# dell-research-harvard/effocr

Hardware: AMD Instinct MI355X
Metric: glyph-crops/sec end-to-end (encode+kNN), 224x224 bs=1024 (higher is better)
Workload: dtype bf16; 1 GPU; BASELINE configs[1]: vit_small_patch16_224 encoder (bf16 MFMA operands, fp32 accumulate/residual/LN/softmax), 1024x3x224x224 fp32 crops per GPU resident in HBM, 10000-row fp32 IndexFlatIP, k=10; seeded random-init weights; crops_per_gpu=1024, global_batch=1024, index_rows=10000, k=10, parallelism=1024 crops per GPU, weights+index replicated

## Files before the change

### effocr_amd/csrc/api.hip

```cpp
#include "../../include/effocr_hip.h"
#include "enc_core.hpp"


#include <math.h>
#include <algorithm>
#include <string.h>
#include <map>
#include <memory>
#include <string>
#include <vector>

namespace effocr {

namespace {

struct Param { std::string name; std::vector<int64_t> shape; int64_t numel; std::vector<float> data; bool set; };

struct VitCfg { int D, depth, heads, mlp; };
struct VitLayerOff { size_t ln1w, ln1b, qkvb, projb, ln2w, ln2b, fc1b, fc2b, qkvw, projw, fc1w, fc2w;
                     size_t qkvw_b, projw_b, fc1w_b, fc2w_b, projw_pp, fc2w_pp, projb_p, fc2b_p, qkvw_bv, qkvb_v;
                     size_t qkvw_bf, qkv_s, qkv_c, fc1w_bf, fc1_s, fc1_c; };
struct ConvSpec { std::string w, bn; int cin, cout, k, stride, pad; size_t w_off, b_off; };
struct CnxBlockOff { size_t dww, dwb, lnw, lnb, w1, b1, w2, b2, gamma; };
struct CnxStageOff { int C, Cp, depth; size_t dslnw, dslnb, dsw, dsb; std::vector<CnxBlockOff> blocks; };

}
}

using namespace effocr;

struct effocr_encoder {
  std::string arch;
  bool is_vit = false;
  int img = 224, prec = PREC_BF16, D = 0;
  std::vector<Param> params;
  std::map<std::string, int> index;
  VitCfg vit{};
  int T = 0, P = 0;
  size_t off_clspos0 = 0, off_pos = 0, off_patchb = 0, off_normw = 0, off_normb = 0, off_patchw = 0, off_patchw_b = 0;
  std::vector<VitLayerOff> layers;
  std::vector<ConvSpec> convs;
  bool is_cnx = false;
  std::vector<CnxStageOff> cnx;
  size_t cnx_stemw = 0, cnx_stemb = 0, cnx_stemlnw = 0, cnx_stemlnb = 0, cnx_headw = 0, cnx_headb = 0;
  bool is_mnv = false;
  MnvNet mnv{};
  size_t wbytes = 0;
  const char* wdev = nullptr;
  int debug = 0;
  int cls_only_last = 1;
  int mlp_stagger_min_rounds = 2;
  int mlp_tail_first = 96;
  int mlp_stagger = 2500;
  int use_projf = 1;
  int use_qkvattn = 1;
  int qa_min_batch = 1;
  int qa_hsplit = 0;
  int use_patchf = 1;
  int use_mlp = 1;
  int use_gemm3 = 1;
  int use_lnfold = 1;
  int tail_split = 1;
  int split6 = 1;
  int pair_parts = 1;
  int mlp_pair = 0;
  int use_blocked = 1;
  int use_gemm2 = 1;
  int panel_rows = 128;
  int use_panel = 1;
  int chunk = 0;
  int call_size_invariant = 0;
  int prof_mode = 0;
  std::string prof_only;
  std::vector<std::pair<hipEvent_t, hipEvent_t>> prof_pool;
  std::vector<std::pair<int, int>> prof_rec;
  std::vector<std::string> prof_names;
  size_t prof_used = 0;
  std::vector<float> prof_ms;
  std::vector<int> prof_cnt;
  std::vector<double> prof_work;
  unsigned long long* prof_clk = nullptr;
  std::vector<double> prof_ghz;
  static constexpr size_t PROF_CLK_SLOTS = 256;
};

namespace effocr {
namespace {

int64_t prod(const std::vector<int64_t>& s) { int64_t p = 1; for (auto v : s) p *= v; return p; }

void add_param(effocr_encoder* e, const std::string& name, std::vector<int64_t> shape) {
  Param p; p.name = name; p.shape = shape; p.numel = prod(shape); p.set = false;
  e->index[name] = (int)e->params.size();
  e->params.push_back(std::move(p));
}

void build_vit(effocr_encoder* e) {
  const int D = e->vit.D, depth = e->vit.depth, mlp = e->vit.mlp;
  e->P = (e->img / 16) * (e->img / 16);
  e->T = e->P + 1;
  add_param(e, "cls_token", {1, 1, D});
  add_param(e, "pos_embed", {1, e->T, D});
  add_param(e, "patch_embed.proj.weight", {D, 3, 16, 16});
  add_param(e, "patch_embed.proj.bias", {D});
  for (int i = 0; i < depth; ++i) {
    const std::string p = "blocks." + std::to_string(i) + ".";
    add_param(e, p + "norm1.weight", {D});
    add_param(e, p + "norm1.bias", {D});
    add_param(e, p + "attn.qkv.weight", {3 * D, D});
    add_param(e, p + "attn.qkv.bias", {3 * D});
    add_param(e, p + "attn.proj.weight", {D, D});
// ... 455 lines not shown
}

struct VitWs { size_t status, x, xn, qkv, att, h, stats, total, rows, hbytes; };
VitWs vit_ws(const effocr_encoder* e, int B) {
  const size_t M = align_up((size_t)B * e->T, 128), D = e->vit.D, es = prec_esize(e->prec);
  Alloc a; VitWs w;
  w.rows = M;
  w.status = a.take(256);
  w.x = a.take(M * D * 4);
  w.xn = a.take(M * D * es);
  w.qkv = a.take(M * 3 * D * es);
  w.att = a.take(M * D * es);
  size_t hb = M * e->vit.mlp * es, pb = (size_t)B * e->P * 768 * es;
  w.hbytes = hb > pb ? hb : pb;
  {
    const size_t cus = (size_t)device_cus(), np = M / 128, tail = np % cus;
    const size_t split = (tail && tail * 6 <= cus) ? 6 : (tail && tail * 4 <= cus) ? 4 : (tail && tail * 2 <= cus) ? 2 : 0;
    const size_t need = split * tail * 128 * D * 4;
    if (need > w.hbytes) w.hbytes = need;
  }
  w.h = a.take(w.hbytes);
  w.stats = a.take(M * 64);
  w.total = a.off;
  return w;
}

int vit_forward(effocr_encoder* e, const void* x, int x16, int B, float* emb, int l2, char* ws, hipStream_t s) {
  const VitWs w = vit_ws(e, B);
  const int D = e->vit.D, T = e->T, Pn = e->P, M = B * T, prec = e->prec;
  const char* wb = e->wdev;
  float* xs = reinterpret_cast<float*>(ws + w.x);
  void* xn = ws + w.xn; void* qkv = ws + w.qkv; void* att = ws + w.att; void* hb = ws + w.h;
  auto F = [&](size_t off) { return reinterpret_cast<const float*>(wb + off); };
  int rc;
  const double Md = (double)M, Dd = (double)D, Hd = (double)e->vit.mlp;
  const bool panel = e->use_panel && panel_gemm_supported(prec, 3 * D, D) && panel_gemm_supported(prec, e->vit.mlp, D);
  const bool g2 = e->use_gemm2 && gemm2_supported(prec, D, e->vit.mlp);
  const bool g2p = e->use_gemm2 && gemm2_supported(prec, D, 768);
  const bool g3all = !panel && e->use_gemm3 && gemm3_supported(prec, 3 * D, D) && gemm3_supported(prec, D, D) &&
                     gemm3_supported(prec, e->vit.mlp, D) && gemm3_supported(prec, D, e->vit.mlp);
  const int blk = (e->use_blocked && g2p && ((panel && g2) || g3all)) ? 1 : 0;
  const bool mlpf = blk && panel && e->use_mlp && mlp_fused_supported(prec, D, e->vit.mlp);
  const bool projf = mlpf && e->use_projf;
  const bool qaf = blk && panel && mlpf && qkv_attn_supported(prec, D, T) && (e->use_qkvattn == 2 || (e->use_qkvattn == 1 && (e->call_size_invariant || B >= e->qa_min_batch)));
  const bool g3 = blk && e->use_gemm3 && gemm3_supported(prec, D, e->vit.mlp);
  const bool patchf = blk && e->use_patchf && patch_embed_fused_supported(prec, D);
  if (!patchf && (rc = timed(e, "im2col_patch16", 0.0, s, [&] { return im2col_patch16(prec, x, x16, B, e->img, e->img, hb, s); }))) return rc;
  int* status = reinterpret_cast<int*>(ws + w.status);
  if (!patchf && (rc = set_cls_rows(F(e->off_clspos0), xs, B, T, D, blk, nullptr, s))) return rc;
  GemmArgs g{};
  if (patchf) {
    PatchArgs pa{};
    pa.x = x; pa.x16 = x16; pa.B = B; pa.H = e->img; pa.W = e->img; pa.Wb = wb + e->off_patchw_b; pa.bias = F(e->off_patchb); pa.pos = F(e->off_pos);
    pa.out = xs; pa.D = D; pa.P = Pn; pa.cls = F(e->off_clspos0);
    if ((rc = timed(e, "patch_embed_fused", 2.0 * B * Pn * Dd * 768.0, s, [&] { return patch_embed_fused(prec, pa, s); }))) return rc;
  } else {
  g.X = hb; g.ldx = 768; g.W = wb + e->off_patchw; g.ldw = 768; g.bias = F(e->off_patchb);
  g.out = xs; g.ldo = D; g.pos = F(e->off_pos); g.M = B * Pn; g.N = D; g.K = 768; g.P = Pn; g.blk_out = blk;
  if ((rc = timed(e, "gemm_patch_embed", 2.0 * B * Pn * Dd * 768.0, s, [&] { return g2p ? gemm2_nt(prec, EPI_PATCH, g, s) : gemm_nt(prec, EPI_PATCH, g, s); }))) return rc;
  }
  const float* cls_x = nullptr;
  bool xn_ready = false;
  for (int i = 0; i < e->vit.depth; ++i) {
    const VitLayerOff& L = e->layers[i];
    if (panel) {
      {
      PanelArgs p{};
      if (qaf) {
        if (!xn_ready && (rc = timed(e, "layernorm", 0.0, s, [&] { return layernorm_rows_blocked(prec, xs, M, D, F(L.ln1w), F(L.ln1b), 1e-6f, xn, s); }))) return rc;
        xn_ready = false;
        QkvAttnArgs q{};
        q.xn = xn; q.Wb = wb + L.qkvw_bv; q.bias = F(L.qkvb_v); q.out = att;
        q.B = B; q.T = T; q.D = D; q.rows_alloc = (int64_t)w.rows; q.hsplit = e->qa_hsplit;
        q.cls_only = (i + 1 == e->vit.depth && e->cls_only_last && projf) ? 1 : 0;
        const bool cls_k = q.cls_only && D == 384 && T > 192;
        const double qa_work = cls_k ? 2.0 * Md * 2.0 * Dd * Dd + 2.0 * (32.0 * B) * Dd * Dd + 4.0 * B * e->vit.heads * 32.0 * T * 64.0
                                     : 2.0 * Md * 3.0 * Dd * Dd + 4.0 * B * e->vit.heads * (double)T * T * 64.0;
        if ((rc = timed(e, "qkv_attn_fused", qa_work, s, [&] { return qkv_attn_fused(prec, q, s); }))) return rc;
      } else {
      p.A = xs; p.lda = D; p.gamma = F(L.ln1w); p.beta = F(L.ln1b); p.eps = 1e-6f; p.W = wb + L.qkvw; p.bias = F(L.qkvb);
      p.out = qkv; p.ldo = 3 * D; p.M = M; p.N = 3 * D; p.K = D; p.rows_padded = 1; p.debug = e->debug; p.panel_rows = e->panel_rows; p.no_tail_split = !e->tail_split;
      p.blk_a = blk; p.blk_out = blk;
      if ((rc = timed(e, "panel_ln_qkv", 2.0 * Md * 3.0 * Dd * Dd, s, [&] { return panel_gemm(prec, PRO_LN, EPI_BIAS, p, s); }))) return rc;
      if ((rc = timed(e, "attention", 4.0 * B * e->vit.heads * (double)T * T * 64.0, s, [&] { return attention(prec, qkv, att, B, T, e->vit.heads, blk, s); }))) return rc;
      }
      if (!projf) {
      p = PanelArgs{};
      p.A = att; p.lda = D; p.W = wb + L.projw; p.bias = F(L.projb); p.out = xs; p.ldo = D; p.resid = xs; p.ldr = D;
      p.M = M; p.N = D; p.K = D; p.rows_padded = 1; p.debug = e->debug; p.panel_rows = e->panel_rows; p.no_tail_split = !e->tail_split; p.blk_a = blk; p.blk_out = blk;
      if ((rc = timed(e, "panel_proj_resid", 2.0 * Md * Dd * Dd, s, [&] { return panel_gemm(prec, PRO_COPY, EPI_BIAS_RESID, p, s); }))) return rc;
      }
      }
      if (mlpf) {
        MlpArgs m{};
        m.x = xs; m.gamma = F(L.ln2w); m.beta = F(L.ln2b); m.eps = 1e-6f; m.W1b = wb + L.fc1w_b; m.b1 = F(L.fc1b);
        m.W2p = wb + L.fc2w_pp; m.b2 = F(L.fc2b_p); m.b2_logical = F(L.fc2b); m.M = M; m.D = D; m.H = e->vit.mlp; m.rows_alloc = (int)w.rows;
        m.partial = reinterpret_cast<float*>(hb); m.partial_bytes = w.hbytes; m.no_tail_split = !e->tail_split; m.no_split6 = !e->split6; m.pair = e->mlp_pair; m.no_pair_parts = !e->pair_parts; m.stagger = e->mlp_stagger; m.stagger_min_rounds = e->mlp_stagger_min_rounds; m.tail_first = e->mlp_tail_first;
        if (e->call_size_invariant) { m.no_tail_split = 1; m.pair = -1; }
        if (projf) {
          m.A = att; m.Wpp = wb + L.projw_pp; m.bp = F(L.projb_p);
          if (i + 1 == e->vit.depth && e->cls_only_last) {
            const size_t Bp = align_up((size_t)B, 128);
            float* xc = reinterpret_cast<float*>(qkv);
            void* ac = static_cast<char*>(qkv) + Bp * D * 4;
            if ((rc = timed(e, "gather_cls", 0.0, s, [&] { return gather_cls_rows_blocked(xs, att, B, T, D, xc, ac, s); }))) return rc;
            m.x = xc; m.A = ac; m.M = B; m.rows_alloc = (int)Bp;
            const double Bd = B;
// ... 363 lines not shown
  auto it = enc->index.find(name);
  if (it == enc->index.end()) return fail(EFFOCR_EINVAL, std::string("set_param: unknown parameter '") + name + "'");
  Param& p = enc->params[it->second];
  if (p.numel != numel)
    return fail(EFFOCR_EINVAL, std::string("set_param: '") + name + "' expects " + std::to_string(p.numel) +
                                   " elements, got " + std::to_string(numel));
  p.data.assign(host, host + numel);
  p.set = true;
  return EFFOCR_OK;
}

size_t effocr_encoder_weights_bytes(const effocr_encoder_t* enc) { return enc ? enc->wbytes : 0; }

int effocr_encoder_upload(effocr_encoder_t* enc, void* weights_dev, size_t bytes) {
  if (!enc || !weights_dev) return fail(EFFOCR_EINVAL, "upload: NULL argument");
  if (bytes < enc->wbytes) return fail(EFFOCR_EWORKSPACE, "upload: weight buffer too small");
  for (const Param& p : enc->params)
    if (!p.set) return fail(EFFOCR_ESTATE, "upload: parameter '" + p.name + "' was never set");
  std::vector<char> blob(enc->wbytes, 0);
  if (enc->is_vit) pack_vit(enc, blob); else if (enc->is_cnx) pack_convnext(enc, blob); else if (enc->is_mnv) pack_mobilenetv3(enc, blob);
  else pack_resnet(enc, blob);
  const hipError_t er = hipMemcpy(weights_dev, blob.data(), enc->wbytes, hipMemcpyHostToDevice);
  if (er != hipSuccess) return fail(EFFOCR_EHIP, std::string("upload: hipMemcpy: ") + hipGetErrorString(er));
  enc->wdev = static_cast<const char*>(weights_dev);
  return EFFOCR_OK;
}

size_t effocr_encoder_workspace_bytes(const effocr_encoder_t* enc, int batch) {
  if (!enc || batch <= 0) return 0;
  if (enc->is_cnx) return convnext_ws(enc, cnx_chunk(enc, batch)).total;
  if (enc->is_mnv) return mnv3_ws(enc, mnv3_chunk(enc, batch)).total;
  if (!enc->is_vit) return resnet_ws(enc, batch).total;
  return vit_ws(enc, (enc->chunk > 0 && enc->chunk < batch) ? enc->chunk : batch).total;
}

int effocr_encoder_set_option(effocr_encoder_t* enc, const char* name, int value) {
  if (!enc || !name) return fail(EFFOCR_EINVAL, "set_option: NULL argument");
  const std::string n = name;
  if (n == "use_panel") { enc->use_panel = value; return EFFOCR_OK; }
  if (n == "debug") { enc->debug = value; return EFFOCR_OK; }
  if (n == "use_gemm2") { enc->use_gemm2 = value; return EFFOCR_OK; }
  if (n == "use_blocked") { enc->use_blocked = value; return EFFOCR_OK; }
  if (n == "tail_split") { enc->tail_split = value; return EFFOCR_OK; }
  if (n == "split6") { enc->split6 = value; return EFFOCR_OK; }
  if (n == "mlp_pair") { enc->mlp_pair = value; return EFFOCR_OK; }
  if (n == "pair_parts") { enc->pair_parts = value; return EFFOCR_OK; }
  if (n == "use_gemm3") { enc->use_gemm3 = value; return EFFOCR_OK; }
  if (n == "use_lnfold") { enc->use_lnfold = value; return EFFOCR_OK; }
  if (n == "use_mlp") { enc->use_mlp = value; return EFFOCR_OK; }
  if (n == "use_qkvattn") { enc->use_qkvattn = value; return EFFOCR_OK; }
  if (n == "qa_min_batch") { enc->qa_min_batch = value; return EFFOCR_OK; }
  if (n == "qa_hsplit") { enc->qa_hsplit = value; return EFFOCR_OK; }
  if (n == "use_patchf") { enc->use_patchf = value; return EFFOCR_OK; }
  if (n == "use_projf") { enc->use_projf = value; return EFFOCR_OK; }
  if (n == "cls_only_last") { enc->cls_only_last = value; return EFFOCR_OK; }
  if (n == "mlp_stagger_min_rounds") { enc->mlp_stagger_min_rounds = value < 1 ? 1 : value; return EFFOCR_OK; }
  if (n == "mlp_tail_first") { enc->mlp_tail_first = value < 0 ? 0 : value & ~7; return EFFOCR_OK; }
  if (n == "mlp_stagger") { enc->mlp_stagger = value < 0 ? 0 : value; return EFFOCR_OK; }
  if (n == "panel_rows") { if (value != 64 && value != 128) return fail(EFFOCR_EINVAL, "set_option: panel_rows must be 64 or 128"); enc->panel_rows = value; return EFFOCR_OK; }
  if (n == "call_size_invariant") {
    if (value != 0 && value != 1) return fail(EFFOCR_EINVAL, "set_option: call_size_invariant must be 0 or 1");
    enc->call_size_invariant = value; return EFFOCR_OK;
  }
  if (n == "chunk") { if (value < 0) return fail(EFFOCR_EINVAL, "set_option: chunk < 0"); enc->chunk = value; return EFFOCR_OK; }
  return fail(EFFOCR_EINVAL, "set_option: unknown option '" + n + "'");
}

int effocr_encoder_set_chunk(effocr_encoder_t* enc, int crops_per_chunk) {
  if (!enc || crops_per_chunk < 0) return fail(EFFOCR_EINVAL, "set_chunk: bad argument");
  enc->chunk = crops_per_chunk;
  return EFFOCR_OK;
}

int effocr_encoder_forward(effocr_encoder_t* enc, const float* x_dev, int batch, float* emb_dev, int l2_normalize,
                           void* workspace_dev, size_t workspace_bytes, void* stream) {
  return effocr_encoder_forward_ex(enc, x_dev, EFFOCR_PREC_FP32, batch, emb_dev, l2_normalize, workspace_dev, workspace_bytes, stream);
}

int effocr_encoder_forward_ex(effocr_encoder_t* enc, const void* x_dev, int x_dtype, int batch, float* emb_dev, int l2_normalize,
                              void* workspace_dev, size_t workspace_bytes, void* stream) {
  if (!enc) return fail(EFFOCR_EINVAL, "forward: NULL encoder");
  if (x_dtype != PREC_FP32 && !(enc->is_vit && enc->prec != PREC_FP32 && x_dtype == enc->prec))
    return fail(x_dtype < 0 || x_dtype > 2 ? EFFOCR_EINVAL : EFFOCR_EUNSUPPORTED,
                "forward: crops must be fp32, or (ViT, 16-bit precision modes) already in the encoder's own operand type");
  const int x16 = x_dtype != PREC_FP32;
  if (batch < 0) return fail(EFFOCR_EINVAL, "forward: negative batch");
  if (batch == 0) return EFFOCR_OK;
  if (!x_dev || !emb_dev || !workspace_dev) return fail(EFFOCR_EINVAL, "forward: NULL device pointer");
  if (!enc->wdev) return fail(EFFOCR_ESTATE, "forward: weights were not uploaded");
  if (workspace_bytes < effocr_encoder_workspace_bytes(enc, batch)) return fail(EFFOCR_EWORKSPACE, "forward: workspace too small");
  if ((int64_t)batch * (enc->is_vit ? enc->T : enc->img * enc->img) >= (int64_t)1 << 30)
    return fail(EFFOCR_EUNSUPPORTED, "forward: batch too large for 32-bit row indices");
  char* ws = static_cast<char*>(workspace_dev);
  if (enc->is_cnx) {
    const int chunk = cnx_chunk(enc, batch);
    const int64_t so = enc->img / 4;
    if ((int64_t)chunk * so * so * 4 * enc->cnx[0].C >= (int64_t)1 << 31)
      return fail(EFFOCR_EUNSUPPORTED, "forward: chunk too large for 32-bit GEMM row indices (effocr_encoder_set_chunk)");
    const size_t img_bytes = (size_t)3 * enc->img * enc->img * 4;
    for (int b0 = 0; b0 < batch; b0 += chunk) {
      const int cb = (batch - b0 < chunk) ? batch - b0 : chunk;
      const int rc = convnext_forward(enc, reinterpret_cast<const float*>(static_cast<const char*>(x_dev) + (size_t)b0 * img_bytes), cb,
                                      emb_dev + (size_t)b0 * enc->D, l2_normalize, ws, S(stream));
      if (rc) return rc;
    }
    return EFFOCR_OK;
// ... 319 lines not shown
```

### effocr_amd/csrc/kernels.hpp

```cpp
#pragma once
#include "common.hpp"

namespace effocr {

enum { PREC_BF16 = 0, PREC_FP16 = 1, PREC_FP32 = 2 };
enum { EPI_BIAS = 0, EPI_BIAS_GELU = 1, EPI_BIAS_RESID = 2, EPI_PATCH = 3,
       EPI_BIAS_SCALE_RESID = 4,
       EPI_BIAS_F32 = 5 };

static inline int prec_esize(int prec) { return prec == PREC_FP32 ? 4 : 2; }

struct GemmArgs {
  const void* X; int64_t ldx;
  const void* W; int64_t ldw;
  const float* bias;
  void* out; int64_t ldo;
  const float* resid; int64_t ldr;
  const float* pos;
  int M, N, K;
  int P;
  int blk_x;
  int blk_out;
  const void* Wblk;
  int rows_alloc;
// ... 5 lines not shown

int gemm_nt(int prec, int epi, const GemmArgs& g, hipStream_t s);

bool gemm2_supported(int prec, int N, int K);
int gemm2_nt(int prec, int epi, const GemmArgs& g, hipStream_t s);

bool gemm3_supported(int prec, int N, int K);
bool gemm3_lnfold_supported(int D);
int gemm3_nt(int prec, int epi, const GemmArgs& g, hipStream_t s);

struct MlpArgs {
  float* x;
  const float* gamma; const float* beta; float eps;
  const void* W1b; const float* b1;
  const void* W2p; const float* b2;
  int M, D, H;
  int rows_alloc;
  float* partial; size_t partial_bytes;
  int no_tail_split;
  int no_split6;
  int no_pair_parts;
  int pair;
  int panel0, tail_rb, stagger_wgs, main_wgs;
  int stagger;
  int stagger_min_rounds;
  int tail_first;
  const void* A; const void* Wpp; const float* bp; const float* b2_logical;
  void* xn_out; const float* gamma_n; const float* beta_n;
};
bool mlp_fused_supported(int prec, int D, int H);
int mlp_fused(int prec, const MlpArgs& a, hipStream_t s);

struct QkvAttnArgs {
  const void* xn;
  const void* Wb; const float* bias;
  void* out;
  int B, T, D;
  int64_t rows_alloc;
  int cls_only;
  int img0;
  int hsplit;
};
bool qkv_attn_supported(int prec, int D, int T);
int qkv_attn_fused(int prec, const QkvAttnArgs& a, hipStream_t s);

struct PatchArgs {
  const void* x; int B, H, W;
  int x16;
  const void* Wb;
  const float* bias; const float* pos;
  const float* cls;
  float* out;
  int D, P;
};
bool patch_embed_fused_supported(int prec, int D);
int patch_embed_fused(int prec, const PatchArgs& a, hipStream_t s);

enum { PRO_COPY = 0, PRO_LN = 1 };
struct PanelArgs {
  const void* A; int64_t lda;
  const float* gamma; const float* beta; float eps;
  const void* W;
  const float* bias;
  void* out; int64_t ldo;
  const float* resid; int64_t ldr;
  int M, N, K;
  unsigned long long* dbg;
  int debug;
  int blk_a;
  int blk_out;
  int panel_rows;
  int rows_padded;
  int no_tail_split;
  int tail_first, tail_split;
};
bool panel_gemm_supported(int prec, int N, int K);
int panel_gemm(int prec, int pro, int epi, const PanelArgs& a, hipStream_t s);

int reduce_layernorm_rows_blocked(int prec_out, float* x, int64_t rows, int D, const float* partial, const float* b2, int nparts, int tail_rb,
                                  int add_x, const float* gamma, const float* beta, float eps, void* out, hipStream_t s);
int layernorm_rows_blocked(int prec_out, const float* x, int64_t rows, int D, const float* gamma, const float* beta,
                           float eps, void* out, hipStream_t s);
int layernorm_rows(int prec_out, const float* x, int64_t rows, int D, const float* gamma, const float* beta,
                   float eps, void* out, hipStream_t s);
int im2col_patch16(int prec_out, const void* x, int x16, int B, int H, int W, void* out, hipStream_t s);
int clock_sample(unsigned long long* out, hipStream_t s);
int set_cls_rows(const float* cls_pos0, float* x, int B, int T, int D, int blocked, int* status_zero, hipStream_t s);
int gather_cls_rows_blocked(const float* x, const void* att, int B, int T, int D, float* xc, void* ac, hipStream_t s);
int attention(int prec, const void* qkv, void* out, int B, int T, int heads, int blocked, hipStream_t s);
int final_cls_norm(const float* x, int B, int T, int D, const float* gamma, const float* beta, float eps,
                   int l2norm, int blocked, float* emb, int* status, hipStream_t s);

size_t knn_workspace_bytes(int64_t B, int64_t N, int D, int k);
int knn_ip_topk(const float* q, int64_t B, const float* xb, int64_t N, int D, int k, float* dist, int64_t* idx,
                void* ws, size_t ws_bytes, hipStream_t s);
size_t knn_screen_workspace_bytes(int64_t B, int64_t N, int D, int k);
void knn_set_wg_target(int n);
void knn_q16_tile(int on);
void knn_two_pass_screen(int on);
void knn_force_tile_kernel(int on);
size_t knn_screen_flag_offset(int64_t B, int64_t N, int D, int k);
int knn_ip_topk_screened(const float* q, int64_t B, const float* xb, const void* xb16, const void* xblk, int64_t N, int D, int k, float xnorm_max,
                         float* dist, int64_t* idx, void* ws, size_t ws_bytes, hipStream_t s);
int convert_bf16_blocked(const float* src, int64_t N, int D, void* dst, hipStream_t s);
void knn_qs_option(int which, int value);
int convert_bf16(const float* src, int64_t n, void* dst, hipStream_t s);
// ... 68 lines not shown
```

### effocr_amd/csrc/patch.hip

```cpp
#include "common.hpp"
#include "kernels.hpp"
#include <type_traits>

constexpr int PE_SLABS = 2;
constexpr int PE_SLABS16 = 4;
#ifndef PATCH_NT
#define PATCH_NT 1
#endif
namespace effocr {
namespace {

template <int I, int N, typename F> __device__ __forceinline__ void pfor(F&& f) {
  if constexpr (I < N) {
    f(std::integral_constant<int, I>{});
    pfor<I + 1, N>(f);
  }
}

constexpr int PE_STAGE = 16384;
constexpr int PE_RING = 8;
constexpr int PE_K = 768;

template <typename E, typename X, int D>
__global__ __launch_bounds__(256, 1) void patch_embed_kernel(PatchArgs a) {
  typedef typename Op16<E>::V8 V8;
  constexpr bool X16 = sizeof(X) == 2;
  constexpr int NSL = X16 ? PE_SLABS16 : PE_SLABS;
  constexpr int KC = PE_K / 8;
  constexpr int OT = D / 32, OG = OT / 4;
  constexpr int KS = PE_K / 64;
  constexpr int NS = KS * OG;
  constexpr int R = PE_RING;
  static_assert(D % 128 == 0 && D <= 384, "patch_embed: a workgroup's output slice must be 128, 256 or 384 wide");
  static_assert(NS >= R - 1, "patch_embed: the panel's stream must be at least as long as the prefetch distance");
  __shared__ __attribute__((aligned(16))) char smem[R * PE_STAGE];
  const int tid = threadIdx.x, lane = tid & 63, r31 = lane & 31, half = lane >> 5;
  const int w = wave_id();
  const int64_t total = (int64_t)a.B * a.P;
  const int nsl = a.D / D;
  const int panel = (int)blockIdx.x / nsl, n0 = ((int)blockIdx.x - panel * nsl) * D;
  const int64_t m = (int64_t)panel * 128 + w * 32 + r31;
  const int64_t mc = m < total ? m : total - 1;
  const int img = (int)(mc / a.P), p = (int)(mc - (int64_t)img * a.P);
  const int PW = a.W / 16, ty = p / PW, tx = p - ty * PW;
  const X* xp = static_cast<const X*>(a.x) + ((int64_t)img * 3 * a.H + ty * 16) * a.W + tx * 16 + 8 * half;
  const int64_t plane = (int64_t)a.H * a.W;

  struct Slab { u32x4 v[X16 ? 4 : 8]; };
  auto load_slab = [&](Slab& sl, int ks) __attribute__((always_inline)) {
#pragma unroll
    for (int c4 = 0; c4 < 4; ++c4) {
      const int kk = ks * 4 + c4;
      const X* q = xp + (int64_t)(kk >> 4) * plane + (int64_t)(kk & 15) * a.W;
      if constexpr (X16) {
        sl.v[c4] = (PATCH_NT & 1) ? __builtin_nontemporal_load(reinterpret_cast<const u32x4*>(q)) : *reinterpret_cast<const u32x4*>(q);
      } else {
        sl.v[2 * c4] = (PATCH_NT & 1) ? __builtin_nontemporal_load(reinterpret_cast<const u32x4*>(q)) : *reinterpret_cast<const u32x4*>(q);
        sl.v[2 * c4 + 1] = (PATCH_NT & 1) ? __builtin_nontemporal_load(reinterpret_cast<const u32x4*>(q + 4)) : *reinterpret_cast<const u32x4*>(q + 4);
      }
    }
  };
  Slab sl[NSL];
#pragma unroll
  for (int i = 0; i < NSL; ++i) load_slab(sl[i], i);
  asm volatile("" ::: "memory");

  const char* Wb = static_cast<const char*>(a.Wb);
  const unsigned lane16 = (unsigned)lane * 16u;
  auto stage_src = [&](int s) __attribute__((always_inline)) -> const char* {
    const int ks = s / OG, g = s - ks * OG;
    return Wb + ((size_t)(4 * g + w + (n0 >> 5)) * KC + 8 * ks) * 512 + lane16;
  };
  const unsigned sW_lds = (unsigned)(size_t)(__attribute__((address_space(3))) char*)smem;
#pragma unroll
  for (int s0 = 0; s0 < R - 1; ++s0) {
    const __attribute__((address_space(1))) void* src = (const __attribute__((address_space(1))) void*)stage_src(s0);
    __attribute__((address_space(3))) void* dst = (__attribute__((address_space(3))) void*)(smem + s0 * PE_STAGE + w * 4096);
    __builtin_amdgcn_global_load_lds(src, dst, 16, 0, 0);
    __builtin_amdgcn_global_load_lds(src, dst, 16, 1024, 0);
    __builtin_amdgcn_global_load_lds(src, dst, 16, 2048, 0);
    __builtin_amdgcn_global_load_lds(src, dst, 16, 3072, 0);
  }
  auto issue_stage_asm = [&](int s) __attribute__((always_inline)) {
    const char* src = stage_src(s);
    const unsigned dst = (unsigned)__builtin_amdgcn_readfirstlane((int)(sW_lds + (unsigned)((s & (R - 1)) * PE_STAGE) + (unsigned)w * 4096u));
    unsigned keep;
    asm volatile("s_mov_b32 %0, m0\n\t"
                 "s_mov_b32 m0, %2\n\t"
                 "s_nop 0\n\t"
                 "global_load_lds_dwordx4 %1, off\n\t"
                 "global_load_lds_dwordx4 %1, off offset:1024\n\t"
                 "global_load_lds_dwordx4 %1, off offset:2048\n\t"
                 "global_load_lds_dwordx4 %1, off offset:3072\n\t"
                 "s_mov_b32 m0, %0"
                 : "=&s"(keep) : "v"(src), "s"(dst) : "memory");
  };

  auto to_frags = [&](const Slab& sl, V8 (&xf)[4]) __attribute__((always_inline)) {
#pragma unroll
    for (int c4 = 0; c4 < 4; ++c4) {
      if constexpr (X16) xf[c4] = __builtin_bit_cast(V8, sl.v[c4]);
      else {
        const f32x4 lo = __builtin_bit_cast(f32x4, sl.v[2 * c4]), hi = __builtin_bit_cast(f32x4, sl.v[2 * c4 + 1]);
        const u32x2 p0 = pack4<E>(lo[0], lo[1], lo[2], lo[3]);
        const u32x2 p1 = pack4<E>(hi[0], hi[1], hi[2], hi[3]);
        const u32x4 q = {p0[0], p0[1], p1[0], p1[1]};
        xf[c4] = __builtin_bit_cast(V8, q);
      }
    }
  };

  f32x16 acc[OT];
#pragma unroll
  for (int t = 0; t < OT; ++t)
#pragma unroll
    for (int r = 0; r < 16; ++r) acc[t][r] = 0.f;

  V8 xf[4];

  const int wo = half * 512 + r31 * 16;
  struct WF { V8 w[4]; };
  WF wf;
  asm volatile("s_waitcnt vmcnt(%0)" ::"n"((R - 2) * 4) : "memory");
  __builtin_amdgcn_s_barrier();
  asm volatile("" ::: "memory");
#pragma unroll
  for (int i = 0; i < 4; ++i) wf.w[i] = *reinterpret_cast<const V8*>(smem + wo + (i * 8) * 512);

  pfor<0, NS>([&](auto S_) {
    constexpr int S = decltype(S_)::value;
    constexpr int ks = S / OG, g = S % OG;
    constexpr bool more = S + R - 1 < NS, next = S + 1 < NS;
    const char* st = smem + (S & (R - 1)) * PE_STAGE;
    const char* stn = smem + ((S + 1) & (R - 1)) * PE_STAGE;
    if constexpr (g == 0) {
      to_frags(sl[ks % NSL], xf);
      if constexpr (ks + NSL < KS) load_slab(sl[ks % NSL], ks + NSL);
    }
    pfor<0, 4>([&](auto C4) {
      constexpr int c4 = decltype(C4)::value;
      if constexpr (c4 == 2) {
        if constexpr (S + R - 2 < NS) asm volatile("s_waitcnt vmcnt(%0)" ::"n"((R - 3) * 4) : "memory");
        else asm volatile("s_waitcnt vmcnt(0)" ::: "memory");
        __builtin_amdgcn_s_barrier();
        asm volatile("" ::: "memory");
      }
      pfor<0, 4>([&](auto I) {
        constexpr int i = decltype(I)::value;
        acc[4 * g + i] = Op16<E>::mfma(wf.w[i], xf[c4], acc[4 * g + i]);
        __builtin_amdgcn_sched_barrier(0);
        if constexpr (c4 < 3) wf.w[i] = *reinterpret_cast<const V8*>(st + wo + (i * 8 + 2 * (c4 + 1)) * 512);
        else if constexpr (next) wf.w[i] = *reinterpret_cast<const V8*>(stn + wo + (i * 8) * 512);
        if constexpr (more && c4 == 2 && i == 0) issue_stage_asm(S + R - 1);
      });
    });
  });

  if (m < total) {
    const int64_t orow = (int64_t)img * (a.P + 1) + 1 + p;
    const float* posr = a.pos + (int64_t)(1 + p) * a.D + n0;
    const float* biasr = a.bias + n0;
    char* ob = reinterpret_cast<char*>(a.out) + ((orow >> 5) * (a.D >> 2) + (n0 >> 2)) * 512 + (orow & 31) * 16;
    pfor<0, OT>([&](auto T_) {
      constexpr int t = decltype(T_)::value;
#pragma unroll
      for (int q = 0; q < 4; ++q) {
        const int f0 = 32 * t + 8 * q + 4 * half;
        const f32x4 bv = *reinterpret_cast<const f32x4*>(biasr + f0);
        const f32x4 pv = *reinterpret_cast<const f32x4*>(posr + f0);
        const f32x4 o = {acc[t][4 * q] + bv[0] + pv[0], acc[t][4 * q + 1] + bv[1] + pv[1], acc[t][4 * q + 2] + bv[2] + pv[2],
                         acc[t][4 * q + 3] + bv[3] + pv[3]};
        if (PATCH_NT & 2) __builtin_nontemporal_store(o, reinterpret_cast<f32x4*>(ob + (f0 >> 2) * 512)); else *reinterpret_cast<f32x4*>(ob + (f0 >> 2) * 512) = o;
      }
    });
    if (a.cls != nullptr && p == 0) {
      const int64_t crow = orow - 1;
      char* cb = reinterpret_cast<char*>(a.out) + ((crow >> 5) * (a.D >> 2) + (n0 >> 2)) * 512 + (crow & 31) * 16;
      for (int c = half; c < D / 4; c += 2)
        *reinterpret_cast<f32x4*>(cb + c * 512) = *reinterpret_cast<const f32x4*>(a.cls + n0 + 4 * c);
    }
  }
}

template <typename E, typename X>
int launch_patch(const PatchArgs& a, hipStream_t s) {
  const int64_t total = (int64_t)a.B * a.P;
  const int64_t panels = (total + 127) / 128;
  if (a.D == 384 && panels * 3 <= device_cus()) {
    hipLaunchKernelGGL((patch_embed_kernel<E, X, 128>), dim3((unsigned)(panels * 3)), dim3(256), 0, s, a);
    return check_launch("patch_embed_fused");
  }
  const int nsl = a.D > 384 ? a.D / 384 : 1;
  const dim3 grid((unsigned)(panels * nsl)), blk(256);
  switch (a.D) {
    case 128: hipLaunchKernelGGL((patch_embed_kernel<E, X, 128>), grid, blk, 0, s, a); break;
    case 256: hipLaunchKernelGGL((patch_embed_kernel<E, X, 256>), grid, blk, 0, s, a); break;
    case 384: case 768: hipLaunchKernelGGL((patch_embed_kernel<E, X, 384>), grid, blk, 0, s, a); break;
    default: return fail(EFFOCR_EUNSUPPORTED, "patch_embed_fused: embed dim must be 128, 256, 384 or 768");
  }
  return check_launch("patch_embed_fused");
}

}

bool patch_embed_fused_supported(int prec, int D) { return (prec == PREC_BF16 || prec == PREC_FP16) && (D == 128 || D == 256 || D == 384 || D == 768); }

int patch_embed_fused(int prec, const PatchArgs& a, hipStream_t s) {
  if (a.B <= 0) return EFFOCR_OK;
  if (!patch_embed_fused_supported(prec, a.D)) return fail(EFFOCR_EUNSUPPORTED, "patch_embed_fused: needs bf16/fp16 and an embed dim of 128, 256, 384 or 768");
  if (a.H % 16 || a.W % 16 || a.P != (a.H / 16) * (a.W / 16)) return fail(EFFOCR_EINVAL, "patch_embed_fused: image size must be a multiple of 16");
  if (a.x16) return prec == PREC_BF16 ? launch_patch<__bf16, __bf16>(a, s) : launch_patch<_Float16, _Float16>(a, s);
  return prec == PREC_BF16 ? launch_patch<__bf16, float>(a, s) : launch_patch<_Float16, float>(a, s);
}

}
```

Measured before the change: 100,800 glyph-crops/s.

## Make fused patch-embed kernel persistent with cross-unit weight and pixel prefetch

Turns the fused patch-embedding GEMM into a persistent kernel with at most one workgroup per CU. Each workgroup loops over panel/slice units, and the LDS weight ring and pixel slab prefetch wrap around into the next unit, so that unit's loads overlap with the current unit's MFMAs and epilogue. The epilogue is restructured to batch bias and position loads, and the CLS-row write becomes a wave-wide ballot loop. Per-launch overhead and pipeline ramp-up are amortised across units, at the cost of more complex vmcnt accounting and fewer resident workgroups. Optional timestamp instrumentation is added behind a compile flag.

```diff
diff --git a/effocr_amd/csrc/api.hip b/effocr_amd/csrc/api.hip
--- a/effocr_amd/csrc/api.hip
+++ b/effocr_amd/csrc/api.hip
@@ -57,6 +57,7 @@
   int qa_min_batch = 1;
   int qa_hsplit = 0;
   int use_patchf = 1;
+  int patch_persist = 1;
   int use_mlp = 1;
   int use_gemm3 = 1;
   int use_lnfold = 1;
@@ -618,7 +619,7 @@
   if (patchf) {
     PatchArgs pa{};
     pa.x = x; pa.x16 = x16; pa.B = B; pa.H = e->img; pa.W = e->img; pa.Wb = wb + e->off_patchw_b; pa.bias = F(e->off_patchb); pa.pos = F(e->off_pos);
-    pa.out = xs; pa.D = D; pa.P = Pn; pa.cls = F(e->off_clspos0);
+    pa.out = xs; pa.D = D; pa.P = Pn; pa.cls = F(e->off_clspos0); pa.persist = e->patch_persist;
     if ((rc = timed(e, "patch_embed_fused", 2.0 * B * Pn * Dd * 768.0, s, [&] { return patch_embed_fused(prec, pa, s); }))) return rc;
   } else {
   g.X = hb; g.ldx = 768; g.W = wb + e->off_patchw; g.ldw = 768; g.bias = F(e->off_patchb);
@@ -1088,6 +1089,7 @@
   if (n == "qa_min_batch") { enc->qa_min_batch = value; return EFFOCR_OK; }
   if (n == "qa_hsplit") { enc->qa_hsplit = value; return EFFOCR_OK; }
   if (n == "use_patchf") { enc->use_patchf = value; return EFFOCR_OK; }
+  if (n == "patch_persist") { enc->patch_persist = value < 0 ? 0 : value; return EFFOCR_OK; }
   if (n == "use_projf") { enc->use_projf = value; return EFFOCR_OK; }
   if (n == "cls_only_last") { enc->cls_only_last = value; return EFFOCR_OK; }
   if (n == "mlp_stagger_min_rounds") { enc->mlp_stagger_min_rounds = value < 1 ? 1 : value; return EFFOCR_OK; }
diff --git a/effocr_amd/csrc/kernels.hpp b/effocr_amd/csrc/kernels.hpp
--- a/effocr_amd/csrc/kernels.hpp
+++ b/effocr_amd/csrc/kernels.hpp
@@ -81,6 +81,7 @@
   const float* cls;
   float* out;
   int D, P;
+  int persist;
 };
 bool patch_embed_fused_supported(int prec, int D);
 int patch_embed_fused(int prec, const PatchArgs& a, hipStream_t s);
diff --git a/effocr_amd/csrc/patch.hip b/effocr_amd/csrc/patch.hip
--- a/effocr_amd/csrc/patch.hip
+++ b/effocr_amd/csrc/patch.hip
@@ -2,7 +2,13 @@
 #include "kernels.hpp"
 #include <type_traits>
 
-constexpr int PE_SLABS = 2;
+#ifndef PE_SLABS_N
+#define PE_SLABS_N 2
+#endif
+#ifndef PE_EPI_TILES
+#define PE_EPI_TILES 2
+#endif
+constexpr int PE_SLABS = PE_SLABS_N;
 constexpr int PE_SLABS16 = 4;
 #ifndef PATCH_NT
 #define PATCH_NT 1
@@ -17,73 +23,115 @@
   }
 }
 
+#ifdef PATCH_STAMP
+constexpr int PE_STAMP_UNITS = 4096, PE_STAMP_N = 16;
+__device__ unsigned long long pe_stamps[PE_STAMP_UNITS * PE_STAMP_N];
+#define PE_STAMP_AT(k) pe_ts[k] = __builtin_amdgcn_s_memtime();
+#else
+#define PE_STAMP_AT(k)
+#endif
+
 constexpr int PE_STAGE = 16384;
 constexpr int PE_RING = 8;
 constexpr int PE_K = 768;
+
+struct PeGeom { int OG, NS, KS, NSL, LPS, R; };
+constexpr int pe_mid_count(PeGeom g, int S) {
+  int n = (g.R - 3) * 4;
+  for (int T = S - (g.R - 3); T <= S; ++T)
+    if (T % g.OG == 0) n += g.LPS;
+  return n < 63 ? n : 63;
+}
+constexpr int pe_slab_count(PeGeom g, int ks) {
+  const int n = (g.NSL - 1) * g.LPS + g.NSL * g.OG * 4;
+  return n < 63 ? n : 63;
+}
 
 template <typename E, typename X, int D>
 __global__ __launch_bounds__(256, 1) void patch_embed_kernel(PatchArgs a) {
   typedef typename Op16<E>::V8 V8;
   constexpr bool X16 = sizeof(X) == 2;
   constexpr int NSL = X16 ? PE_SLABS16 : PE_SLABS;
+  constexpr int LPS = X16 ? 4 : 8;
   constexpr int KC = PE_K / 8;
   constexpr int OT = D / 32, OG = OT / 4;
   constexpr int KS = PE_K / 64;
   constexpr int NS = KS * OG;
   constexpr int R = PE_RING;
+  constexpr PeGeom GEO{OG, NS, KS, NSL, LPS, R};
   static_assert(D % 128 == 0 && D <= 384, "patch_embed: a workgroup's output slice must be 128, 256 or 384 wide");
   static_assert(NS >= R - 1, "patch_embed: the panel's stream must be at least as long as the prefetch distance");
+  static_assert(KS % NSL == 0, "patch_embed: slab ks lives in buffer ks % NSL, also across units");
   __shared__ __attribute__((aligned(16))) char smem[R * PE_STAGE];
   const int tid = threadIdx.x, lane = tid & 63, r31 = lane & 31, half = lane >> 5;
   const int w = wave_id();
+#ifdef PATCH_STAMP
+  unsigned long long pe_ts[6] = {}, pe_vm = 0, pe_bar = 0;
+  unsigned long long pe_rt0 = __builtin_amdgcn_s_memrealtime();
+  int pe_ord = 0;
+#endif
+  PE_STAMP_AT(0)
   const int64_t total = (int64_t)a.B * a.P;
   const int nsl = a.D / D;
-  const int panel = (int)blockIdx.x / nsl, n0 = ((int)blockIdx.x - panel * nsl) * D;
-  const int64_t m = (int64_t)panel * 128 + w * 32 + r31;
-  const int64_t mc = m < total ? m : total - 1;
-  const int img = (int)(mc / a.P), p = (int)(mc - (int64_t)img * a.P);
-  const int PW = a.W / 16, ty = p / PW, tx = p - ty * PW;
-  const X* xp = static_cast<const X*>(a.x) + ((int64_t)img * 3 * a.H + ty * 16) * a.W + tx * 16 + 8 * half;
+  const int nunits = (int)((total + 127) / 128) * nsl;
+  const int PW = a.W / 16;
   const int64_t plane = (int64_t)a.H * a.W;
+  struct Loc { int n0; int64_t m; int img, p; const X* xp; };
+  auto locate = [&](int unit) __attribute__((always_inline)) -> Loc {
+    Loc l;
+    const int panel = unit / nsl;
+    l.n0 = (unit - panel * nsl) * D;
+    l.m = (int64_t)panel * 128 + w * 32 + r31;
+    const int64_t mc = l.m < total ? l.m : total - 1;
+    l.img = (int)(mc / a.P); l.p = (int)(mc - (int64_t)l.img * a.P);
+    const int ty = l.p / PW, tx = l.p - ty * PW;
+    l.xp = static_cast<const X*>(a.x) + ((int64_t)l.img * 3 * a.H + ty * 16) * a.W + tx * 16 + 8 * half;
+    return l;
+  };
+  int unit = (int)blockIdx.x;
+  Loc cur = locate(unit);
+  const X* xp = cur.xp;
 
   struct Slab { u32x4 v[X16 ? 4 : 8]; };
+  auto ldpix = [&](u32x4& d, const X* q, auto OFF) __attribute__((always_inline)) {
+    if constexpr (decltype(OFF)::value == 0) {
+      if constexpr (PATCH_NT & 1) asm volatile("global_load_dwordx4 %0, %1, off nt" : "=v"(d) : "v"(q) : "memory");
+      else asm volatile("global_load_dwordx4 %0, %1, off" : "=v"(d) : "v"(q) : "memory");
+    } else {
+      if constexpr (PATCH_NT & 1) asm volatile("global_load_dwordx4 %0, %1, off offset:16 nt" : "=v"(d) : "v"(q) : "memory");
+      else asm volatile("global_load_dwordx4 %0, %1, off offset:16" : "=v"(d) : "v"(q) : "memory");
+    }
+  };
   auto load_slab = [&](Slab& sl, int ks) __attribute__((always_inline)) {
 #pragma unroll
     for (int c4 = 0; c4 < 4; ++c4) {
       const int kk = ks * 4 + c4;
       const X* q = xp + (int64_t)(kk >> 4) * plane + (int64_t)(kk & 15) * a.W;
-      if constexpr (X16) {
-        sl.v[c4] = (PATCH_NT & 1) ? __builtin_nontemporal_load(reinterpret_cast<const u32x4*>(q)) : *reinterpret_cast<const u32x4*>(q);
-      } else {
-        sl.v[2 * c4] = (PATCH_NT & 1) ? __builtin_nontemporal_load(reinterpret_cast<const u32x4*>(q)) : *reinterpret_cast<const u32x4*>(q);
-        sl.v[2 * c4 + 1] = (PATCH_NT & 1) ? __builtin_nontemporal_load(reinterpret_cast<const u32x4*>(q + 4)) : *reinterpret_cast<const u32x4*>(q + 4);
-      }
-    }
+      if constexpr (X16) ldpix(sl.v[c4], q, std::integral_constant<int, 0>{});
+      else {
+        ldpix(sl.v[2 * c4], q, std::integral_constant<int, 0>{});
+        ldpix(sl.v[2 * c4 + 1], q, std::integral_constant<int, 1>{});
+      }
+    }
+  };
+  auto tie_slab = [&](Slab& sl) __attribute__((always_inline)) {
+#pragma unroll
+    for (int c = 0; c < (X16 ? 4 : 8); ++c) asm volatile("" : "+v"(sl.v[c]));
   };
   Slab sl[NSL];
 #pragma unroll
   for (int i = 0; i < NSL; ++i) load_slab(sl[i], i);
-  asm volatile("" ::: "memory");
 
   const char* Wb = static_cast<const char*>(a.Wb);
   const unsigned lane16 = (unsigned)lane * 16u;
-  auto stage_src = [&](int s) __attribute__((always_inline)) -> const char* {
+  auto unit_src = [&](int n0_) __attribute__((always_inline)) -> const char* { return Wb + (size_t)(w + (n0_ >> 5)) * KC * 512 + lane16; };
+  const char* wsrc = unit_src(cur.n0);
+  int sb = 0;
+  const unsigned sW_lds = (unsigned)(size_t)(__attribute__((address_space(3))) char*)smem;
+  auto issue_stage_asm = [&](int s, int slot) __attribute__((always_inline)) {
     const int ks = s / OG, g = s - ks * OG;
-    return Wb + ((size_t)(4 * g + w + (n0 >> 5)) * KC + 8 * ks) * 512 + lane16;
-  };
-  const unsigned sW_lds = (unsigned)(size_t)(__attribute__((address_space(3))) char*)smem;
-#pragma unroll
-  for (int s0 = 0; s0 < R - 1; ++s0) {
-    const __attribute__((address_space(1))) void* src = (const __attribute__((address_space(1))) void*)stage_src(s0);
-    __attribute__((address_space(3))) void* dst = (__attribute__((address_space(3))) void*)(smem + s0 * PE_STAGE + w * 4096);
-    __builtin_amdgcn_global_load_lds(src, dst, 16, 0, 0);
-    __builtin_amdgcn_global_load_lds(src, dst, 16, 1024, 0);
-    __builtin_amdgcn_global_load_lds(src, dst, 16, 2048, 0);
-    __builtin_amdgcn_global_load_lds(src, dst, 16, 3072, 0);
-  }
-  auto issue_stage_asm = [&](int s) __attribute__((always_inline)) {
-    const char* src = stage_src(s);
-    const unsigned dst = (unsigned)__builtin_amdgcn_readfirstlane((int)(sW_lds + (unsigned)((s & (R - 1)) * PE_STAGE) + (unsigned)w * 4096u));
+    const char* src = wsrc + ((size_t)(4 * g) * KC + 8 * ks) * 512;
+    const unsigned dst = (unsigned)__builtin_amdgcn_readfirstlane((int)(sW_lds + (unsigned)(slot * PE_STAGE) + (unsigned)w * 4096u));
     unsigned keep;
     asm volatile("s_mov_b32 %0, m0\n\t"
                  "s_mov_b32 m0, %2\n\t"
@@ -95,6 +143,8 @@
                  "s_mov_b32 m0, %0"
                  : "=&s"(keep) : "v"(src), "s"(dst) : "memory");
   };
+#pragma unroll
+  for (int s0 = 0; s0 < R - 1; ++s0) issue_stage_asm(s0, s0);
 
   auto to_frags = [&](const Slab& sl, V8 (&xf)[4]) __attribute__((always_inline)) {
 #pragma unroll
@@ -111,87 +161,185 @@
   };
 
   f32x16 acc[OT];
-#pragma unroll
-  for (int t = 0; t < OT; ++t)
-#pragma unroll
-    for (int r = 0; r < 16; ++r) acc[t][r] = 0.f;
-
   V8 xf[4];
-
   const int wo = half * 512 + r31 * 16;
   struct WF { V8 w[4]; };
   WF wf;
-  asm volatile("s_waitcnt vmcnt(%0)" ::"n"((R - 2) * 4) : "memory");
-  __builtin_amdgcn_s_barrier();
-  asm volatile("" ::: "memory");
-#pragma unroll
-  for (int i = 0; i < 4; ++i) wf.w[i] = *reinterpret_cast<const V8*>(smem + wo + (i * 8) * 512);
-
-  pfor<0, NS>([&](auto S_) {
-    constexpr int S = decltype(S_)::value;
-    constexpr int ks = S / OG, g = S % OG;
-    constexpr bool more = S + R - 1 < NS, next = S + 1 < NS;
-    const char* st = smem + (S & (R - 1)) * PE_STAGE;
-    const char* stn = smem + ((S + 1) & (R - 1)) * PE_STAGE;
-    if constexpr (g == 0) {
-      to_frags(sl[ks % NSL], xf);
-      if constexpr (ks + NSL < KS) load_slab(sl[ks % NSL], ks + NSL);
-    }
-    pfor<0, 4>([&](auto C4) {
-      constexpr int c4 = decltype(C4)::value;
-      if constexpr (c4 == 2) {
-        if constexpr (S + R - 2 < NS) asm volatile("s_waitcnt vmcnt(%0)" ::"n"((R - 3) * 4) : "memory");
-        else asm volatile("s_waitcnt vmcnt(0)" ::: "memory");
-        __builtin_amdgcn_s_barrier();
-        asm volatile("" ::: "memory");
-      }
-      pfor<0, 4>([&](auto I) {
-        constexpr int i = decltype(I)::value;
-        acc[4 * g + i] = Op16<E>::mfma(wf.w[i], xf[c4], acc[4 * g + i]);
-        __builtin_amdgcn_sched_barrier(0);
-        if constexpr (c4 < 3) wf.w[i] = *reinterpret_cast<const V8*>(st + wo + (i * 8 + 2 * (c4 + 1)) * 512);
-        else if constexpr (next) wf.w[i] = *reinterpret_cast<const V8*>(stn + wo + (i * 8) * 512);
-        if constexpr (more && c4 == 2 && i == 0) issue_stage_asm(S + R - 1);
+  asm volatile("s_waitcnt vmcnt(0)" ::: "memory");
+#pragma unroll
+  for (int i = 0; i < NSL; ++i) tie_slab(sl[i]);
+  PE_STAMP_AT(1)
+
+  for (;;) {
+    __builtin_amdgcn_s_barrier();
+    asm volatile("" ::: "memory");
+    PE_STAMP_AT(2)
+    const int un = unit + (int)gridDim.x;
+    const bool has_next = un < nunits;
+#pragma unroll
+    for (int i = 0; i < 4; ++i) wf.w[i] = *reinterpret_cast<const V8*>(smem + (sb & (R - 1)) * PE_STAGE + wo + (i * 8) * 512);
+
+    pfor<0, NS>([&](auto S_) {
+      constexpr int S = decltype(S_)::value;
+      constexpr int ks = S / OG, g = S % OG;
+      constexpr bool next = S + 1 < NS;
+      const char* st = smem + ((sb + S) & (R - 1)) * PE_STAGE;
+      const char* stn = smem + ((sb + S + 1) & (R - 1)) * PE_STAGE;
+      if constexpr (S == NS - (R - 1)) {
+        wsrc = unit_src(has_next ? (un % nsl) * D : cur.n0);
+      }
+      if constexpr (g == 0) {
+        if constexpr (ks >= NSL) {
+          asm volatile("s_waitcnt vmcnt(%0)" ::"n"(pe_slab_count(GEO, ks)) : "memory");
+          tie_slab(sl[ks % NSL]);
+        }
+        to_frags(sl[ks % NSL], xf);
+        if constexpr (ks + NSL == KS) {
+          xp = has_next ? locate(un).xp : static_cast<const X*>(a.x);
+        }
+        if constexpr (ks + NSL < KS) load_slab(sl[ks % NSL], ks + NSL);
+        else load_slab(sl[ks % NSL], ks + NSL - KS);
+      }
+      pfor<0, 4>([&](auto C4) {
+        constexpr int c4 = decltype(C4)::value;
+        if constexpr (c4 == 2) {
+#ifdef PATCH_STAMP
+          const unsigned long long t0_ = __builtin_amdgcn_s_memtime();
+#endif
+          if constexpr (S >= R - 2) asm volatile("s_waitcnt vmcnt(%0)" ::"n"(pe_mid_count(GEO, S)) : "memory");
+#ifdef PATCH_STAMP
+          const unsigned long long t1_ = __builtin_amdgcn_s_memtime();
+#endif
+          __builtin_amdgcn_s_barrier();
+          asm volatile("" ::: "memory");
+#ifdef PATCH_STAMP
+          const unsigned long long t2_ = __builtin_amdgcn_s_memtime();
+          pe_vm += t1_ - t0_; pe_bar += t2_ - t1_;
+#endif
+        }
+        pfor<0, 4>([&](auto I) {
+          constexpr int i = decltype(I)::value;
+          if constexpr (ks == 0 && c4 == 0) {
+            const f32x16 z = {0.f, 0.f, 0.f, 0.f, 0.f, 0.f, 0.f, 0.f, 0.f, 0.f, 0.f, 0.f, 0.f, 0.f, 0.f, 0.f};
+            acc[4 * g + i] = Op16<E>::mfma(wf.w[i], xf[c4], z);
+          } else {
+            acc[4 * g + i] = Op16<E>::mfma(wf.w[i], xf[c4], acc[4 * g + i]);
+          }
+          __builtin_amdgcn_sched_barrier(0);
+          if constexpr (c4 < 3) wf.w[i] = *reinterpret_cast<const V8*>(st + wo + (i * 8 + 2 * (c4 + 1)) * 512);
+          else if constexpr (next) wf.w[i] = *reinterpret_cast<const V8*>(stn + wo + (i * 8) * 512);
+          if constexpr (c4 == 2 && i == 0) issue_stage_asm((S + R - 1) % NS, (sb + S + R - 1) & (R - 1));
+        });
       });
     });
-  });
-
-  if (m < total) {
-    const int64_t orow = (int64_t)img * (a.P + 1) + 1 + p;
-    const float* posr = a.pos + (int64_t)(1 + p) * a.D + n0;
-    const float* biasr = a.bias + n0;
-    char* ob = reinterpret_cast<char*>(a.out) + ((orow >> 5) * (a.D >> 2) + (n0 >> 2)) * 512 + (orow & 31) * 16;
-    pfor<0, OT>([&](auto T_) {
-      constexpr int t = decltype(T_)::value;
-#pragma unroll
-      for (int q = 0; q < 4; ++q) {
-        const int f0 = 32 * t + 8 * q + 4 * half;
-        const f32x4 bv = *reinterpret_cast<const f32x4*>(biasr + f0);
-        const f32x4 pv = *reinterpret_cast<const f32x4*>(posr + f0);
-        const f32x4 o = {acc[t][4 * q] + bv[0] + pv[0], acc[t][4 * q + 1] + bv[1] + pv[1], acc[t][4 * q + 2] + bv[2] + pv[2],
-                         acc[t][4 * q + 3] + bv[3] + pv[3]};
-        if (PATCH_NT & 2) __builtin_nontemporal_store(o, reinterpret_cast<f32x4*>(ob + (f0 >> 2) * 512)); else *reinterpret_cast<f32x4*>(ob + (f0 >> 2) * 512) = o;
-      }
-    });
-    if (a.cls != nullptr && p == 0) {
-      const int64_t crow = orow - 1;
-      char* cb = reinterpret_cast<char*>(a.out) + ((crow >> 5) * (a.D >> 2) + (n0 >> 2)) * 512 + (crow & 31) * 16;
-      for (int c = half; c < D / 4; c += 2)
-        *reinterpret_cast<f32x4*>(cb + c * 512) = *reinterpret_cast<const f32x4*>(a.cls + n0 + 4 * c);
-    }
+    PE_STAMP_AT(3)
+
+    {
+      const bool ok = cur.m < total;
+      const int img = cur.img, p = cur.p, n0 = cur.n0;
+      const int64_t orow = (int64_t)img * (a.P + 1) + 1 + p;
+      const float* posr = a.pos + (int64_t)(1 + p) * a.D + n0 + 4 * half;
+      const float* biasr = a.bias + n0 + 4 * half;
+      char* ob = reinterpret_cast<char*>(a.out) + ((orow >> 5) * (a.D >> 2) + (n0 >> 2)) * 512 + (orow & 31) * 16 + half * 512;
+      constexpr int BT = OT % PE_EPI_TILES == 0 ? PE_EPI_TILES : 2;
+      static_assert(OT % BT == 0, "patch_embed: the epilogue's batches are whole tiles");
+      pfor<0, OT / BT>([&](auto B_) {
+        constexpr int b = decltype(B_)::value;
+        f32x4 bv[BT * 4], pv[BT * 4];
+#pragma unroll
+        for (int j = 0; j < BT * 4; ++j) {
+          const int f0 = 32 * (b * BT + j / 4) + 8 * (j % 4);
+          bv[j] = *reinterpret_cast<const f32x4*>(biasr + f0);
+          pv[j] = *reinterpret_cast<const f32x4*>(posr + f0);
+        }
+        asm volatile("" ::: "memory");
+        if constexpr (b == 0) {
+          asm volatile("s_waitcnt vmcnt(0)" ::: "memory");
+#pragma unroll
+          for (int i = 0; i < NSL; ++i) tie_slab(sl[i]);
+        }
+        f32x4 o[BT * 4];
+#pragma unroll
+        for (int j = 0; j < BT * 4; ++j) {
+          asm volatile("" : "+v"(bv[j]), "+v"(pv[j]));
+          const int t = b * BT + j / 4, q = j % 4;
+          o[j] = f32x4{acc[t][4 * q] + bv[j][0] + pv[j][0], acc[t][4 * q + 1] + bv[j][1] + pv[j][1], acc[t][4 * q + 2] + bv[j][2] + pv[j][2],
+                       acc[t][4 * q + 3] + bv[j][3] + pv[j][3]};
+        }
+        if (ok) {
+#pragma unroll
+          for (int j = 0; j < BT * 4; ++j) {
+            f32x4* dst = reinterpret_cast<f32x4*>(ob + (8 * (b * BT + j / 4) + 2 * (j % 4)) * 512);
+            if (PATCH_NT & 2) __builtin_nontemporal_store(o[j], dst); else *dst = o[j];
+          }
+        }
+#ifdef PATCH_STAMP
+        if constexpr (b == 0) { asm volatile("" ::: "memory"); PE_STAMP_AT(4) }
+#endif
+        asm volatile("" ::: "memory");
+      });
+      if (a.cls != nullptr) {
+        unsigned long long todo = __builtin_amdgcn_ballot_w64(ok && p == 0 && half == 0);
+        while (todo) {
+          const int l = __builtin_ctzll(todo);
+          todo &= todo - 1;
+          const int64_t crow = (int64_t)(((unsigned long long)(unsigned)__builtin_amdgcn_readlane((int)((unsigned long long)orow >> 32), l) << 32) |
+                                         (unsigned)__builtin_amdgcn_readlane((int)orow, l)) - 1;
+          char* cb = reinterpret_cast<char*>(a.out) + ((crow >> 5) * (a.D >> 2) + (n0 >> 2)) * 512 + (crow & 31) * 16;
+          constexpr int NP = (D / 4 + 63) / 64;
+          f32x4 cv[NP];
+#pragma unroll
+          for (int k = 0; k < NP; ++k) {
+            const int c = lane + 64 * k;
+            cv[k] = *reinterpret_cast<const f32x4*>(a.cls + n0 + 4 * (c < D / 4 ? c : 0));
+          }
+#pragma unroll
+          for (int k = 0; k < NP; ++k) asm volatile("" : "+v"(cv[k]));
+#pragma unroll
+          for (int k = 0; k < NP; ++k) {
+            const int c = lane + 64 * k;
+            if (c < D / 4) *reinterpret_cast<f32x4*>(cb + c * 512) = cv[k];
+          }
+        }
+      }
+    }
+#ifdef PATCH_STAMP
+    asm volatile("" ::: "memory");
+    PE_STAMP_AT(5)
+    if (w == 0 && unit < PE_STAMP_UNITS) {
+      unsigned long long* row = pe_stamps + (size_t)unit * PE_STAMP_N;
+#pragma unroll
+      for (int k = 0; k < 6; ++k) row[k] = pe_ts[k];
+      row[6] = pe_vm; row[7] = pe_bar;
+      row[8] = __builtin_amdgcn_s_getreg((4 << 0) | (0 << 6) | (31 << 11)) | ((unsigned long long)__builtin_amdgcn_s_getreg((20 << 0) | (0 << 6) | (31 << 11)) << 32);
+      row[9] = pe_rt0; row[10] = __builtin_amdgcn_s_memrealtime(); row[11] = blockIdx.x; row[12] = pe_ord;
+    }
+    pe_vm = 0; pe_bar = 0; ++pe_ord;
+    pe_rt0 = __builtin_amdgcn_s_memrealtime();
+    PE_STAMP_AT(0)
+    pe_ts[1] = pe_ts[0];
+#endif
+    if (!has_next) break;
+    unit = un;
+    cur = locate(unit);
+    sb = (sb + NS) & (R - 1);
   }
+  asm volatile("s_waitcnt vmcnt(0)" ::: "memory");
 }
 
 template <typename E, typename X>
 int launch_patch(const PatchArgs& a, hipStream_t s) {
   const int64_t total = (int64_t)a.B * a.P;
   const int64_t panels = (total + 127) / 128;
-  if (a.D == 384 && panels * 3 <= device_cus()) {
+  const int cus = device_cus();
+  if (a.D == 384 && panels * 3 <= cus && a.persist < 2) {
     hipLaunchKernelGGL((patch_embed_kernel<E, X, 128>), dim3((unsigned)(panels * 3)), dim3(256), 0, s, a);
     return check_launch("patch_embed_fused");
   }
   const int nsl = a.D > 384 ? a.D / 384 : 1;
-  const dim3 grid((unsigned)(panels * nsl)), blk(256);
+  const int64_t units = panels * nsl;
+  const int64_t cap = a.persist >= 2 ? a.persist : a.persist == 1 ? cus : units;
+  const dim3 grid((unsigned)(units > cap ? cap : units)), blk(256);
   switch (a.D) {
     case 128: hipLaunchKernelGGL((patch_embed_kernel<E, X, 128>), grid, blk, 0, s, a); break;
     case 256: hipLaunchKernelGGL((patch_embed_kernel<E, X, 256>), grid, blk, 0, s, a); break;
@@ -214,3 +362,9 @@
 }
 
 }
+#ifdef PATCH_STAMP
+extern "C" int effocr_debug_patch_stamps(unsigned long long* out, int n) {
+  (void)hipDeviceSynchronize();
+  return (int)hipMemcpyFromSymbol(out, HIP_SYMBOL(effocr::pe_stamps), (size_t)n * sizeof(unsigned long long));
+}
+#endif
```

Result: no change. 101,400 glyph-crops/s (median of 6 runs) (+0.6%).
